# sjtuytc/UnboundedNeRFPytorch

Hardware: AMD Instinct MI355X
Metric: Msamples/sec (Mip-360 garden-shaped 1920x1080x256 frame, FourierGrid render) (higher is better)
Workload: dtype f32; 1 GPU; S1 1920x1080x256 G200 F3(P7) C12 rgbnet 39-128-128-3 f32 stepsize 1.31 thres 1e-4 white-noise grids; rays=2073600, samples_per_ray=256, chunks_per_frame=1, parallelism=1 GPU, step=ray generation + march + shade + un-tiling to image order; 3 frames in flight

## Files before the change

unboundednerfpytorch_amd/csrc/ugrid_march.hip:

```cpp
#include "ugrid_render.h"
#include "ugrid_rays.h"

__global__ void k_pack_bricks(const float *__restrict__ grid, int P, int C, int X, int Y, int Z, int H,
                              int CH, int coef, float *__restrict__ out, int64_t total) {
  for (int64_t o = (int64_t)blockIdx.x * blockDim.x + threadIdx.x; o < total;
       o += (int64_t)gridDim.x * blockDim.x) {
    int64_t q = o;
    int ch, c;
    if (H == 2) {
      const int qi = (int)(q % (8 * CH)); q /= (8 * CH);
      c = (qi >> 1) & 7;
      ch = (qi >> 4) * 2 + (qi & 1);
    } else {
      ch = (int)(q % CH); q /= CH;
      c = (int)(q % 8); q /= 8;
    }
    const int h = (int)(q % H); q /= H;
    const int k = (int)(q % (Z - 1)); q /= (Z - 1);
    const int j = (int)(q % (Y - 1)); q /= (Y - 1);
    const int i = (int)(q % (X - 1)); q /= (X - 1);
    const int l = (int)q;
    const int chan = h * CH + ch;
    float v = 0.f;
    if (chan < C) {
// ... 703 lines not shown
extern "C" int ugrid_train_sample(const float *density_grid, int P, int X, int Y, int Z, int freq_num, const float *rays_o,
                                  const float *rays_d, int64_t n_rays, const float *t_table, int32_t n_samples,
                                  const float *scene_center3, const float *scene_radius3, const float *xyz_min,
                                  const float *xyz_max, double bg_len, int norm_l2, float act_shift, float interval,
                                  float thres, float *scratch_pts, float *scratch_density, int32_t *scratch_step,
                                  float *scratch_w, float *scratch_T, int32_t *count, int32_t *count2, float *alphainv_last,
                                  ugrid_stream_t s) {
  if (!scratch_w || !scratch_T || !count2 || !alphainv_last) return (int)hipErrorInvalidValue;
  return ug_train_march_any(density_grid, P, X, Y, Z, freq_num, rays_o, rays_d, n_rays, t_table, n_samples, scene_center3, scene_radius3,
                            xyz_min, xyz_max, bg_len, norm_l2, act_shift, interval, thres, scratch_pts, scratch_density, scratch_step,
                            count, scratch_w, scratch_T, count2, alphainv_last, s);
}

extern "C" int ugrid_train_sample_compact(int64_t n_rays, int32_t n_samples, float act_shift, float interval, float thres,
                                          const float *scratch_pts, const float *scratch_density, const int32_t *scratch_step,
                                          const float *scratch_w, const float *scratch_T, const int32_t *count,
                                          const int64_t *offset_end, const int32_t *count2, const int64_t *offset_end2,
                                          const float *t_table, float *pts1, float *density1, float *weights1, float *T1,
                                          int32_t *pos2, float *pts2, float *density2, float *alpha2, float *weights2,
                                          int64_t *ray_id2, int64_t *step_id2, float *t2, ugrid_stream_t s) {
  if (n_rays <= 0) return 0;
  hipLaunchKernelGGL(k_train_compact2, dim3(ug_blocks(n_rays * UG_WAVE, 256)), dim3(256), 0, ST(s), n_rays, n_samples, act_shift, interval,
                     thres, scratch_pts, scratch_density, scratch_step, scratch_w, scratch_T, count, offset_end, count2, offset_end2,
                     t_table, pts1, density1, weights1, T1, pos2, pts2, density2, alpha2, weights2, ray_id2, step_id2, t2,
                     (uint8_t *)nullptr, ug_tl_devn.cap > 0 ? ug_tl_devn.cap : INT64_MAX);
  UG_LAUNCH_CHECK();
  return 0;
}

static int ug_fill_train_vox(ug_train_vox *v, const uint8_t *mask, const int32_t *mask_dims3, const float *xyz2ijk_scale3,
                             const float *xyz2ijk_shift3) {
  if (!mask_dims3) return (int)hipErrorInvalidValue;
  v->dist_thres = 0.f; v->near = 0.f; v->far = 0.f; v->stepdist = 1.f;
  v->plane_shift = nullptr; v->D = 1;
  return ug_fill_mask_args(*v, mask, mask_dims3[0], mask_dims3[1], mask_dims3[2], xyz2ijk_scale3, xyz2ijk_shift3);
}

extern "C" int ugrid_train_sample_dcvgo(const float *density_grid, int X, int Y, int Z, const float *rays_o, const float *rays_d,
                                        int64_t n_rays, const float *t_table, int32_t n_samples, const float *scene_center3,
                                        const float *scene_radius3, const float *xyz_min, const float *xyz_max, double bg_len,
                                        int norm_l2, float dist_thres, const uint8_t *mask, const int32_t *mask_dims3,
                                        const float *xyz2ijk_scale3, const float *xyz2ijk_shift3, float act_shift, float interval,
                                        float thres, float *scratch_pts, float *scratch_density, int32_t *scratch_step,
                                        float *scratch_w, float *scratch_T, int32_t *count, int32_t *count2, float *alphainv_last,
                                        ugrid_stream_t s) {
  if (n_rays <= 0) return 0;
  if (n_samples <= 0 || !scratch_w || !scratch_T || !count2 || !alphainv_last || !t_table) return (int)hipErrorInvalidValue;
  ug_train_vox v;
  const int rc = ug_fill_train_vox(&v, mask, mask_dims3, xyz2ijk_scale3, xyz2ijk_shift3);
  if (rc) return rc;
  v.dist_thres = dist_thres;
  ug_train_args a;
  a.n_rays = n_rays; a.S = n_samples; a.P = 1; a.F = 0; a.X = X; a.Y = Y; a.Z = Z; a.norm_l2 = norm_l2;
  a.cx = scene_center3[0]; a.cy = scene_center3[1]; a.cz = scene_center3[2];
  a.rx = scene_radius3[0]; a.ry = scene_radius3[1]; a.rz = scene_radius3[2];
  const double Bd = 1.0 + bg_len;
  a.B = (float)Bd; a.A = (float)bg_len;
  a.shift = act_shift; a.interval = interval; a.thres = thres;
  hipLaunchKernelGGL(HIP_KERNEL_NAME(k_train_march_vox<1>), dim3(ug_blocks(n_rays * UG_WAVE, 256)), dim3(256), 0, ST(s), a, v, density_grid,
                     rays_o, rays_d, t_table, xyz_min, xyz_max, scratch_pts, scratch_density, scratch_step, count, scratch_w, scratch_T,
                     count2, alphainv_last);
  UG_LAUNCH_CHECK();
  return 0;
}

extern "C" int ugrid_train_sample_dvgo(const float *density_grid, int X, int Y, int Z, const float *rays_o, const float *rays_d,
                                       int64_t n_rays, int32_t slots_per_ray, const float *xyz_min, const float *xyz_max, float near,
                                       float far, float stepdist, const uint8_t *mask, const int32_t *mask_dims3,
                                       const float *xyz2ijk_scale3, const float *xyz2ijk_shift3, float act_shift, float interval,
                                       float thres, float *scratch_pts, float *scratch_density, int32_t *scratch_step,
                                       float *scratch_w, float *scratch_T, int32_t *count, int32_t *count2, float *alphainv_last,
                                       ugrid_stream_t s) {
  if (n_rays <= 0) return 0;
  if (slots_per_ray <= 0 || !(stepdist > 0.f) || !scratch_w || !scratch_T || !count2 || !alphainv_last) return (int)hipErrorInvalidValue;
  ug_train_vox v;
  const int rc = ug_fill_train_vox(&v, mask, mask_dims3, xyz2ijk_scale3, xyz2ijk_shift3);
  if (rc) return rc;
  v.near = near; v.far = far; v.stepdist = stepdist;
  ug_train_args a;
  a.n_rays = n_rays; a.S = slots_per_ray; a.P = 1; a.F = 0; a.X = X; a.Y = Y; a.Z = Z; a.norm_l2 = 0;
  a.cx = a.cy = a.cz = 0.f; a.rx = a.ry = a.rz = 1.f; a.B = 1.f; a.A = 0.f;
  a.shift = act_shift; a.interval = interval; a.thres = thres;
  hipLaunchKernelGGL(HIP_KERNEL_NAME(k_train_march_vox<2>), dim3(ug_blocks(n_rays * UG_WAVE, 256)), dim3(256), 0, ST(s), a, v, density_grid,
                     rays_o, rays_d, (const float *)nullptr, xyz_min, xyz_max, scratch_pts, scratch_density, scratch_step, count, scratch_w,
                     scratch_T, count2, alphainv_last);
  UG_LAUNCH_CHECK();
  return 0;
}

extern "C" int ugrid_train_sample_mpi(const float *density_grid, int X, int Y, int Z, const float *rays_o, const float *rays_d,
                                      int64_t n_rays, int32_t n_steps, const float *xyz_min, const float *xyz_max,
                                      const float *act_shift, int32_t mpi_depth, const uint8_t *mask, const int32_t *mask_dims3,
                                      const float *xyz2ijk_scale3, const float *xyz2ijk_shift3, float interval, float thres,
                                      float *scratch_pts, float *scratch_density, int32_t *scratch_step, float *scratch_w,
                                      float *scratch_T, int32_t *count, int32_t *count2, float *alphainv_last, ugrid_stream_t s) {
  if (n_rays <= 0) return 0;
  if (n_steps < 2 || !act_shift || mpi_depth < 1 || mpi_depth > 256 || !scratch_w || !scratch_T || !count2 || !alphainv_last)
    return (int)hipErrorInvalidValue;
  ug_train_vox v;
  const int rc = ug_fill_train_vox(&v, mask, mask_dims3, xyz2ijk_scale3, xyz2ijk_shift3);
  if (rc) return rc;
  v.plane_shift = act_shift; v.D = mpi_depth;
  ug_train_args a;
  a.n_rays = n_rays; a.S = n_steps; a.P = 1; a.F = 0; a.X = X; a.Y = Y; a.Z = Z; a.norm_l2 = 0;
  a.cx = a.cy = a.cz = 0.f; a.rx = a.ry = a.rz = 1.f; a.B = 1.f; a.A = 0.f;
  a.shift = 0.f; a.interval = interval; a.thres = thres;
  hipLaunchKernelGGL(HIP_KERNEL_NAME(k_train_march_vox<3>), dim3(ug_blocks(n_rays * UG_WAVE, 256)), dim3(256), 0, ST(s), a, v, density_grid,
                     rays_o, rays_d, (const float *)nullptr, xyz_min, xyz_max, scratch_pts, scratch_density, scratch_step, count, scratch_w,
                     scratch_T, count2, alphainv_last);
  UG_LAUNCH_CHECK();
  return 0;
}

extern "C" int ugrid_train_sample_compact_vox(int64_t n_rays, int32_t slots_per_ray, float act_shift, float interval, float thres,
                                              const float *scratch_pts, const float *scratch_density, const int32_t *scratch_step,
                                              const float *scratch_w, const float *scratch_T, const int32_t *count,
                                              const int64_t *offset_end, const int32_t *count2, const int64_t *offset_end2,
                                              const float *t_table, float *pts1, float *density1, float *weights1, float *T1,
                                              int32_t *pos2, float *pts2, float *density2, float *alpha2, float *weights2,
                                              int64_t *ray_id2, int64_t *step_id2, float *t2, uint8_t *inner2, ugrid_stream_t s) {
  if (n_rays <= 0) return 0;
  hipLaunchKernelGGL(k_train_compact2, dim3(ug_blocks(n_rays * UG_WAVE, 256)), dim3(256), 0, ST(s), n_rays, slots_per_ray, act_shift,
                     interval, thres, scratch_pts, scratch_density, scratch_step, scratch_w, scratch_T, count, offset_end, count2,
                     offset_end2, t_table, pts1, density1, weights1, T1, pos2, pts2, density2, alpha2, weights2, ray_id2, step_id2, t2,
                     inner2, ug_tl_devn.cap > 0 ? ug_tl_devn.cap : INT64_MAX);
  UG_LAUNCH_CHECK();
  return 0;
}

extern "C" int ugrid_train_sample_backward(int64_t n_rays, float act_shift, float interval, const float *density1,
                                           const float *weights1, const float *T1, const int32_t *pos2, const int32_t *count,
                                           const int64_t *offset_end, const float *alphainv_last, const float *g_weights2,
                                           const float *g_alphainv_last, const float *g_density2, float *g_density1,
                                           ugrid_stream_t s) {
  if (n_rays <= 0) return 0;
  hipLaunchKernelGGL(k_train_sample_bwd, dim3(ug_blocks(n_rays * UG_WAVE, 256)), dim3(256), 0, ST(s), n_rays, act_shift, interval,
                     density1, weights1, T1, pos2, count, offset_end, alphainv_last, g_weights2, g_alphainv_last, g_density2, g_density1);
  UG_LAUNCH_CHECK();
  return 0;
}

extern "C" int ugrid_train_compact(int64_t n_rays, int32_t n_samples, const float *scratch_pts, const float *scratch_density,
                                   const int32_t *scratch_step, const int32_t *count, const int64_t *offset_end,
                                   const float *t_table, float *pts, float *density, int64_t *ray_id, int64_t *step_id,
                                   float *t, ugrid_stream_t s) {
  if (n_rays <= 0) return 0;
  hipLaunchKernelGGL(k_train_compact, dim3(ug_blocks(n_rays * UG_WAVE, 256)), dim3(256), 0, ST(s), n_rays, n_samples,
                     scratch_pts, scratch_density, scratch_step, count, offset_end, t_table, pts, density, ray_id, step_id, t);
  UG_LAUNCH_CHECK();
  return 0;
}

template <class MarchTile>
__device__ __forceinline__ void ug_march_block(const ug_ws_view &ws, int64_t nblocks, MarchTile march) {
  const int64_t blk = ug_xcd_remap(blockIdx.x, nblocks);
  if (blk >= nblocks) return;
  const int64_t tile = blk * 4 + (threadIdx.x >> 6);
  if (tile >= ws.n_tiles) return;
  const int n = march(tile, ws.ent + tile * ws.cap, ws.slot + tile * ws.cap);
  if (ug_lane() == 0) ws.count[tile] = n;
}

struct ug_march_geom { ug_ws_view ws; int64_t nblocks; dim3 grid; };
static inline ug_march_geom ug_march_geometry(void *ws_mem, int64_t n_rays, int32_t S) {
  ug_march_geom g;
  g.ws = ug_ws_make(ws_mem, n_rays, S);
  g.nblocks = (g.ws.n_tiles + 3) / 4;
  g.grid = dim3((unsigned)(((g.nblocks + 7) / 8) * 8));
  return g;
}

template <int F, bool L2, int W>
__global__ void __launch_bounds__(256, W)
k_march(ug_march_args a, const float *__restrict__ rays_o, const float *__restrict__ rays_d,
        const float *__restrict__ t_table, const float *__restrict__ s_table,
        const float *__restrict__ bricks, float *__restrict__ alphainv_last, float *__restrict__ depth,
        ug_ws_view ws, int64_t nblocks) {
  ug_march_block(ws, nblocks, [&](int64_t tile, float4 *ent, uint8_t *slot) {
    return ug_march_tile<F, L2>(a, rays_o, rays_d, t_table, s_table, bricks, alphainv_last, depth, tile, ent, slot);
  });
}


template <bool L2>
__global__ void __launch_bounds__(256, 5)
k_march_dcvgo(ug_march_args a, ug_dc_args dc, const float *__restrict__ rays_o, const float *__restrict__ rays_d,
              const float *__restrict__ t_table, const float *__restrict__ s_table, const float *__restrict__ bricks,
              float *__restrict__ alphainv_last, float *__restrict__ depth, float *__restrict__ wsum_mid, ug_ws_view ws,
              int64_t nblocks) {
  ug_march_block(ws, nblocks, [&](int64_t tile, float4 *ent, uint8_t *slot) {
    return ug_march_tile<0, L2, true>(a, rays_o, rays_d, t_table, s_table, bricks, alphainv_last, depth, tile, ent, slot, dc, wsum_mid);
  });
}

__global__ void __launch_bounds__(256, 6)
k_march_dvgo(ug_march_args a, ug_dv_args dv, const float *__restrict__ rays_o, const float *__restrict__ rays_d,
             const float *__restrict__ bricks, float *__restrict__ alphainv_last, float *__restrict__ depth, ug_ws_view ws,
             int64_t nblocks) {
  ug_march_block(ws, nblocks, [&](int64_t tile, float4 *ent, uint8_t *slot) {
    return ug_march_tile_dvgo(a, dv, rays_o, rays_d, bricks, alphainv_last, depth, tile, ent, slot, a.S);
  });
}

__global__ void __launch_bounds__(256, 6)
k_march_mpi(ug_march_args a, ug_mpi_args mp, const float *__restrict__ rays_o, const float *__restrict__ rays_d,
            const float *__restrict__ bricks, const float *__restrict__ act_shift, float *__restrict__ alphainv_last,
            float *__restrict__ depth, ug_ws_view ws, int64_t nblocks) {
  __shared__ float shift[256];
  if ((int)threadIdx.x < mp.D) shift[threadIdx.x] = act_shift[threadIdx.x];
  __syncthreads();
  ug_march_block(ws, nblocks, [&](int64_t tile, float4 *ent, uint8_t *slot) {
    return ug_march_tile_mpi(a, mp, rays_o, rays_d, bricks, shift, alphainv_last, depth, tile, ent, slot);
  });
}

extern "C" int64_t ugrid_render_ws_bytes(int64_t n_rays, int32_t S) {
  const int64_t n_tiles = (n_rays + UG_WAVE - 1) / UG_WAVE, cap = (int64_t)UG_WAVE * S;
  return 256 + ug_align256(n_tiles * 4) + ug_align256(n_tiles * cap * 16) + ug_align256(n_tiles * cap);
}

static int ug_grid_query_any(bool cl, const float *grid, int P, int C, int X, int Y, int Z, const float *xyz,
                             const float *xyz_min, const float *xyz_max, int freq_num, int64_t n, float *out, hipStream_t st) {
  if (n <= 0) return 0;
  if (P != (freq_num > 0 ? 2 * freq_num + 1 : 1)) return (int)hipErrorInvalidValue;
  const int64_t nl = ug_launch_rows(n);
  if (cl)
    hipLaunchKernelGGL(HIP_KERNEL_NAME(k_grid_query<true>), dim3(ug_blocks(nl * C, 256)), dim3(256), 0, st, grid, P, C, X, Y, Z, xyz,
                       xyz_min, xyz_max, freq_num, n, out, ug_tl_devn.ptr);
  else
    hipLaunchKernelGGL(HIP_KERNEL_NAME(k_grid_query<false>), dim3(ug_blocks(nl, 256)), dim3(256), 0, st, grid, P, C, X, Y, Z, xyz,
                       xyz_min, xyz_max, freq_num, n, out, ug_tl_devn.ptr);
  UG_LAUNCH_CHECK();
  return 0;
}

extern "C" int ugrid_grid_query(const float *grid, int P, int C, int X, int Y, int Z, const float *xyz,
                                const float *xyz_min, const float *xyz_max, int freq_num, int64_t n,
                                float *out, ugrid_stream_t s) {
  return ug_grid_query_any(false, grid, P, C, X, Y, Z, xyz, xyz_min, xyz_max, freq_num, n, out, ST(s));
}

extern "C" int ugrid_grid_query_cl(const float *grid, int P, int C, int X, int Y, int Z, const float *xyz,
                                   const float *xyz_min, const float *xyz_max, int freq_num, int64_t n,
                                   float *out, ugrid_stream_t s) {
  return ug_grid_query_any(true, grid, P, C, X, Y, Z, xyz, xyz_min, xyz_max, freq_num, n, out, ST(s));
}

static int ug_grid_query_backward_any(bool cl, const float *grad_out, int P, int C, int X, int Y, int Z, const float *xyz,
                                      const float *xyz_min, const float *xyz_max, int freq_num, int64_t n,
                                      float *grad_grid, hipStream_t st, uint32_t *touch = nullptr) {
  if (n <= 0) return 0;
  if (P != (freq_num > 0 ? 2 * freq_num + 1 : 1)) return (int)hipErrorInvalidValue;
  const int64_t nl = ug_launch_rows(n);
  if (cl)
    hipLaunchKernelGGL(HIP_KERNEL_NAME(k_grid_query_backward<true>), dim3(ug_blocks(nl * P * C, 256)), dim3(256), 0, st, grad_out, P, C,
                       X, Y, Z, xyz, xyz_min, xyz_max, freq_num, n, grad_grid, touch, ug_tl_devn.ptr);
  else
    hipLaunchKernelGGL(HIP_KERNEL_NAME(k_grid_query_backward<false>), dim3(ug_blocks(nl * P, 256)), dim3(256), 0, st, grad_out, P, C,
                       X, Y, Z, xyz, xyz_min, xyz_max, freq_num, n, grad_grid, (uint32_t *)nullptr, ug_tl_devn.ptr);
  UG_LAUNCH_CHECK();
  return 0;
}

extern "C" int ugrid_grid_query_backward(const float *grad_out, int P, int C, int X, int Y, int Z, const float *xyz,
                                         const float *xyz_min, const float *xyz_max, int freq_num, int64_t n,
                                         float *grad_grid, ugrid_stream_t s) {
  return ug_grid_query_backward_any(false, grad_out, P, C, X, Y, Z, xyz, xyz_min, xyz_max, freq_num, n, grad_grid, ST(s));
}

extern "C" int ugrid_grid_query_backward_cl(const float *grad_out, int P, int C, int X, int Y, int Z, const float *xyz,
                                            const float *xyz_min, const float *xyz_max, int freq_num, int64_t n,
                                            float *grad_grid, ugrid_stream_t s) {
  return ug_grid_query_backward_any(true, grad_out, P, C, X, Y, Z, xyz, xyz_min, xyz_max, freq_num, n, grad_grid, ST(s));
}

extern "C" int ugrid_grid_query_backward_cl_touch(const float *grad_out, int P, int C, int X, int Y, int Z, const float *xyz,
                                                  const float *xyz_min, const float *xyz_max, int freq_num, int64_t n,
                                                  float *grad_grid, uint32_t *touch, ugrid_stream_t s) {
  return ug_grid_query_backward_any(true, grad_out, P, C, X, Y, Z, xyz, xyz_min, xyz_max, freq_num, n, grad_grid, ST(s), touch);
}

extern "C" int ugrid_count_views_accumulate(const float *rays_o, const float *rays_d, int64_t n_rays, const float *xyz_min,
                                            const float *xyz_max, float near, float far, float stepdist, int32_t n_samples, int X, int Y,
                                            int Z, float *acc, ugrid_stream_t s) {
  if (n_rays <= 0 || n_samples <= 0) return 0;
  if (!rays_o || !rays_d || !xyz_min || !xyz_max || !acc || X < 1 || Y < 1 || Z < 1) return (int)hipErrorInvalidValue;
  hipLaunchKernelGGL(k_count_views_accumulate, dim3(ug_blocks(n_rays, 64)), dim3(64), 0, ST(s), rays_o, rays_d, n_rays, xyz_min, xyz_max,
                     near, far, stepdist, n_samples, X, Y, Z, acc);
  UG_LAUNCH_CHECK();
  return 0;
}

extern "C" int ugrid_count_views_commit(float *acc, float *count, int64_t n, ugrid_stream_t s) {
  if (n <= 0) return 0;
  if (!acc || !count) return (int)hipErrorInvalidValue;
  const int64_t blocks = ug_blocks(n, 256);
  hipLaunchKernelGGL(k_count_views_commit, dim3((unsigned)(blocks < 65536 ? blocks : 65536)), dim3(256), 0, ST(s), acc, count, n);
  UG_LAUNCH_CHECK();
  return 0;
}

static inline int ug_brick_ch(int C, int *H) {
  if (C == 1) { *H = 1; return 1; }
  *H = 2;
  return UG_CH(C);
}

extern "C" int64_t ugrid_brick_bytes(int P, int C, int X, int Y, int Z, int direct) {
  int H, CH = ug_brick_ch(C, &H);
  if (direct) { H = 1; CH = 4; }
  return (int64_t)P * (X - 1) * (Y - 1) * (Z - 1) * H * 8 * CH * (int64_t)sizeof(float);
}

extern "C" int ugrid_pack_bricks(const float *grid, int P, int C, int X, int Y, int Z, int direct,
                                 float *bricks, ugrid_stream_t s) {
  if (X < 2 || Y < 2 || Z < 2 || P < 1 || C < 1) return (int)hipErrorInvalidValue;
  int H, CH = ug_brick_ch(C, &H);
  if (direct) { H = 1; CH = 4; }
  const int64_t total = (int64_t)P * (X - 1) * (Y - 1) * (Z - 1) * H * 8 * CH;
  int64_t blocks = (total + 255) / 256;
  if (blocks > 256 * 64) blocks = 256 * 64;
  if (C == 12 && !direct) {
    if (P > 1 && (int64_t)(X - 1) * (Y - 1) * (Z - 1) * 384 >= ((int64_t)1 << 32)) return (int)hipErrorInvalidValue;
    hipLaunchKernelGGL(k_pack_quad, dim3((unsigned)blocks), dim3(256), 0, ST(s), grid, P, C, X, Y, Z, bricks, total);
    UG_LAUNCH_CHECK();
    return 0;
  }
  int coef = direct ? 0 : 1;
  hipLaunchKernelGGL(k_pack_bricks, dim3((unsigned)blocks), dim3(256), 0, ST(s), grid, P, C, X, Y, Z, H, CH,
                     coef, bricks, total);
  UG_LAUNCH_CHECK();
  return 0;
}

static int g_march_waves = 6;
extern "C" int ug_set_march_waves(int w) { if (w < 4 || w > 6) return 1; g_march_waves = w; return 0; }

template <int F, int W>
static int ug_march_launch_w(const ugrid_render_params *p, const ug_march_args &a, const float *rays_o,
                             const float *rays_d, const float *t_table, const float *s_table,
                             const float *bricks, float *alphainv_last, float *depth, const ug_march_geom &g,
                             hipStream_t st) {
  if (p->norm_l2)
    hipLaunchKernelGGL(HIP_KERNEL_NAME(k_march<F, true, W>), g.grid, dim3(256), 0, st, a, rays_o,
                       rays_d, t_table, s_table, bricks, alphainv_last, depth, g.ws, g.nblocks);
  else
    hipLaunchKernelGGL(HIP_KERNEL_NAME(k_march<F, false, W>), g.grid, dim3(256), 0, st, a, rays_o,
                       rays_d, t_table, s_table, bricks, alphainv_last, depth, g.ws, g.nblocks);
  UG_LAUNCH_CHECK();
  return 0;
}

template <int F>
static int ug_march_launch(const ugrid_render_params *p, const ug_march_args &a, const float *rays_o,
                           const float *rays_d, const float *t_table, const float *s_table,
                           const float *bricks, float *alphainv_last, float *depth, const ug_march_geom &g,
                           hipStream_t st) {
  switch (g_march_waves) {
    case 4: return ug_march_launch_w<F, 4>(p, a, rays_o, rays_d, t_table, s_table, bricks, alphainv_last, depth, g, st);
    case 6: return ug_march_launch_w<F, 6>(p, a, rays_o, rays_d, t_table, s_table, bricks, alphainv_last, depth, g, st);
    default: return ug_march_launch_w<F, 5>(p, a, rays_o, rays_d, t_table, s_table, bricks, alphainv_last, depth, g, st);
  }
}

extern "C" int ugrid_render_march(const ugrid_render_params *p, const float *rays_o, const float *rays_d,
// ... 81 lines not shown
```

unboundednerfpytorch_amd/csrc/ugrid_render.h:

```cpp
#pragma once
#include "ugrid_common.h"
#include "ugrid_math.h"
#include <string.h>

#define UG_CH(C) (2 * (((C) + 3) / 4))
#define UG_MAX_F 5


typedef float f32x16 __attribute__((ext_vector_type(16)));

struct ug_vec3 { float x, y, z; };

__device__ __forceinline__ float ug_norm3_torch(float x, float y, float z) {
  return sqrtf(fmaf(z, z, fmaf(y, y, x * x)));
}

template <bool L2>
__device__ __forceinline__ ug_vec3 ug_contract(ug_vec3 p, float B, float A) {
  const float nrm = L2 ? ug_norm3_torch(p.x, p.y, p.z) : fmaxf(fabsf(p.x), fmaxf(fabsf(p.y), fabsf(p.z)));
  if (!(nrm <= 1.0f)) {
    const float sc = B - (1.0f / nrm) * A;
    p.x = p.x / nrm * sc;
    p.y = p.y / nrm * sc;
    p.z = p.z / nrm * sc;
// ... 4 lines not shown
struct ug_axis { int cell; float wlo, whi; };

__device__ __forceinline__ ug_axis ug_axis_setup(float c, int n) {
  const float ix = ((c + 1.f) / 2.f) * (float)(n - 1);
  const float f0 = floorf(ix);
  ug_axis a;
  float wlo = (f0 + 1.f) - ix;
  float whi = ix - f0;
  int i0 = (int)fminf(fmaxf(f0, -2.f), (float)n);
  if (i0 < 0 || i0 > n - 1) wlo = 0.f;
  if (i0 + 1 < 0 || i0 + 1 > n - 1) whi = 0.f;
  if (i0 < 0) {
    a.cell = 0; a.wlo = (i0 == -1) ? whi : 0.f; a.whi = 0.f;
  } else if (i0 > n - 2) {
    a.cell = n - 2; a.whi = (i0 == n - 1) ? wlo : 0.f; a.wlo = 0.f;
  } else {
    a.cell = i0; a.wlo = wlo; a.whi = whi;
  }
  return a;
}

struct ug_cellw { int64_t rec; float w[8]; };

__device__ __forceinline__ ug_cellw ug_cell_setup(float ux, float uy, float uz, int X, int Y, int Z,
                                                 int64_t level_base) {
  const ug_axis ax = ug_axis_setup(ux, X), ay = ug_axis_setup(uy, Y), az = ug_axis_setup(uz, Z);
  ug_cellw r;
  r.rec = level_base + ((int64_t)ax.cell * (Y - 1) + ay.cell) * (Z - 1) + az.cell;
  r.w[0] = az.wlo * ay.wlo * ax.wlo;
  r.w[1] = az.whi * ay.wlo * ax.wlo;
  r.w[2] = az.wlo * ay.whi * ax.wlo;
  r.w[3] = az.whi * ay.whi * ax.wlo;
  r.w[4] = az.wlo * ay.wlo * ax.whi;
  r.w[5] = az.whi * ay.wlo * ax.whi;
  r.w[6] = az.wlo * ay.whi * ax.whi;
  r.w[7] = az.whi * ay.whi * ax.whi;
  return r;
}

template <int F>
struct ug_levels { float cx[2 * F + 1], cy[2 * F + 1], cz[2 * F + 1]; };

template <int F>
__device__ __forceinline__ ug_levels<F> ug_pe(float ux, float uy, float uz) {
  ug_levels<F> L;
  L.cx[0] = ux; L.cy[0] = uy; L.cz[0] = uz;
#pragma unroll
  for (int k = 0; k < F; ++k) {
    const float f = (float)(1 << k);
    float s, c;
    sincosf(f * ux, &s, &c); L.cx[2 * k + 1] = s; L.cx[2 * k + 2] = c;
    sincosf(f * uy, &s, &c); L.cy[2 * k + 1] = s; L.cy[2 * k + 2] = c;
    sincosf(f * uz, &s, &c); L.cz[2 * k + 1] = s; L.cz[2 * k + 2] = c;
  }
  return L;
}

__device__ __forceinline__ float ug_unorm(float p, float lo, float hi) {
  return ((p - lo) / (hi - lo)) * 2.f - 1.f;
}

struct ug_ws_view {
  int32_t *count;
  float4 *ent;
  uint8_t *slot;
  int64_t n_tiles, cap;
};
#define UG_FEAT_STRIDE 12

__host__ __device__ static inline int64_t ug_align256(int64_t x) { return (x + 255) & ~(int64_t)255; }

static inline ug_ws_view ug_ws_make(void *ws, int64_t n_rays, int32_t S) {
  ug_ws_view v;
  v.n_tiles = (n_rays + UG_WAVE - 1) / UG_WAVE;
  v.cap = (int64_t)UG_WAVE * S;
  char *b = (char *)ws + 256;
  v.count = (int32_t *)b;
  b += ug_align256(v.n_tiles * (int64_t)sizeof(int32_t));
  v.ent = (float4 *)b;
  b += ug_align256(v.n_tiles * v.cap * (int64_t)sizeof(float4));
  v.slot = (uint8_t *)b;
  return v;
}

__device__ __forceinline__ int64_t ug_xcd_remap(int64_t b, int64_t nblocks) {
  const int64_t per = (nblocks + 7) / 8;
  return (b % 8) * per + b / 8;
}

struct ug_march_args {
  int64_t n_rays;
  int32_t S, X, Y, Z;
  float cx, cy, cz, rx, ry, rz;
  float lox, loy, loz, hix, hiy, hiz;
  float ex, ey, ez, irx, iry, irz;
  float B, A;
  float shift, interval, thres;
};

__device__ __forceinline__ float ug_density_level(const char *__restrict__ lvl, float cx, float cy, float cz,
                                                  int X, int Y, int Z) {
  const ug_axis_fast ax = ug_axis_inrange(cx, X), ay = ug_axis_inrange(cy, Y), az = ug_axis_inrange(cz, Z);
  const unsigned row = (unsigned)fmaf(ax.cellf, (float)(Y - 1), ay.cellf);
  const unsigned off = __umul24(row, (unsigned)(Z - 1) << 5) + ((unsigned)az.cell << 5);
  const float4 *b = (const float4 *)(lvl + off);
  const float4 v0 = b[0], v1 = b[1];
  const float tz = az.whi, ty = ay.whi, tx = ax.whi;
  const float p00 = fmaf(v0.y, tz, v0.x), p01 = fmaf(v0.w, tz, v0.z);
  const float p10 = fmaf(v1.y, tz, v1.x), p11 = fmaf(v1.w, tz, v1.z);
  return fmaf(fmaf(p11, ty, p10), tx, fmaf(p01, ty, p00));
}

__device__ __forceinline__ void ug_normalise(const ug_march_args &a, float px, float py, float pz, float &ux, float &uy, float &uz) {
  ux = ug_div_r(px - a.lox, a.ex, a.irx) * 2.f - 1.f;
  uy = ug_div_r(py - a.loy, a.ey, a.iry) * 2.f - 1.f;
  uz = ug_div_r(pz - a.loz, a.ez, a.irz) * 2.f - 1.f;
}

__device__ __forceinline__ bool ug_outside_box(const ug_march_args &a, float px, float py, float pz) {
  return (a.lox > px) | (a.loy > py) | (a.loz > pz) | (a.hix < px) | (a.hiy < py) | (a.hiz < pz);
}

struct ug_mask_args {
  const uint8_t *mask;
  int32_t mi, mj, mk;
  float sx, sy, sz, hx, hy, hz;
};

__device__ __forceinline__ bool ug_mask_lookup(const ug_mask_args &m, float px, float py, float pz) {
  float fi = roundf(px * m.sx + m.hx), fj = roundf(py * m.sy + m.hy), fk = roundf(pz * m.sz + m.hz);
  fi = (fi != fi) ? 0.f : fi; fj = (fj != fj) ? 0.f : fj; fk = (fk != fk) ? 0.f : fk;
  if (fi >= 0.f && fi < (float)m.mi && fj >= 0.f && fj < (float)m.mj && fk >= 0.f && fk < (float)m.mk)
    return m.mask[((int64_t)fi * m.mj + (int64_t)fj) * m.mk + (int64_t)fk] != 0;
  return false;
}

static inline int ug_fill_mask_args(ug_mask_args &m, const uint8_t *mask, int32_t mask_x, int32_t mask_y, int32_t mask_z,
                                    const float *scale3, const float *shift3) {
  if (!mask || !scale3 || !shift3 || mask_x < 1 || mask_y < 1 || mask_z < 1) return (int)hipErrorInvalidValue;
  m.mask = mask; m.mi = mask_x; m.mj = mask_y; m.mk = mask_z;
  m.sx = scale3[0]; m.sy = scale3[1]; m.sz = scale3[2];
  m.hx = shift3[0]; m.hy = shift3[1]; m.hz = shift3[2];
  return 0;
}

__device__ __forceinline__ bool ug_composite(float alpha, float thres, float &T, float &w, bool &done) {
  if (!(alpha > thres)) return false;
  w = T * alpha;
  T = (float)((double)T * (1. - (double)alpha));
  if ((double)T < 1e-3) done = true;
  return w > thres;
}

__device__ __forceinline__ void ug_append_survivors(bool surv, float px, float py, float pz, float w, int lane,
                                                    float4 *__restrict__ ent, uint8_t *__restrict__ slot, int &nsurv) {
  const unsigned long long m = __ballot(surv);
  if (m != 0ull) {
    if (surv) {
      const int idx = nsurv + __builtin_amdgcn_mbcnt_hi((unsigned)(m >> 32), __builtin_amdgcn_mbcnt_lo((unsigned)m, 0u));
      ent[idx] = make_float4(px, py, pz, w);
      slot[idx] = (uint8_t)lane;
    }
    nsurv += __popcll(m);
  }
}

struct ug_dc_args : ug_mask_args {
  float dist_thres;
};

template <int F, bool L2, bool DC = false>
__device__ __forceinline__ int ug_march_tile(const ug_march_args &a, const float *__restrict__ rays_o,
                                             const float *__restrict__ rays_d, const float *__restrict__ t_table,
                                             const float *__restrict__ s_table, const float *__restrict__ bricks,
                                             float *__restrict__ alphainv_last, float *__restrict__ depth,
                                             int64_t tile, float4 *__restrict__ ent, uint8_t *__restrict__ slot,
                                             const ug_dc_args &dc = ug_dc_args{}, float *__restrict__ wsum_mid = nullptr) {
  constexpr int P = 2 * F + 1;
  const int lane = ug_lane();
  const int64_t ray = tile * UG_WAVE + lane;
  const bool valid = ray < a.n_rays;

  float ox = 0.f, oy = 0.f, oz = 0.f, dx = 0.f, dy = 0.f, dz = 1.f;
  if (valid) {
    const float rox = rays_o[3 * ray], roy = rays_o[3 * ray + 1], roz = rays_o[3 * ray + 2];
    const float rdx = rays_d[3 * ray], rdy = rays_d[3 * ray + 1], rdz = rays_d[3 * ray + 2];
    ox = (rox - a.cx) / a.rx; oy = (roy - a.cy) / a.ry; oz = (roz - a.cz) / a.rz;
    const float dn = ug_norm3_torch(rdx, rdy, rdz);
    dx = rdx / dn; dy = rdy / dn; dz = rdz / dn;
  }

  const size_t lvl_bytes = (size_t)(a.X - 1) * (a.Y - 1) * (a.Z - 1) * 32;
  const char *__restrict__ bkb = (const char *)bricks;

  float T = 1.f, dsum = 0.f;
  bool done = !valid;
  int nsurv = 0;
  [[maybe_unused]] float cum = 0.f, ppx = 0.f, ppy = 0.f, ppz = 0.f, wmid = 0.f;

  for (int j = 0; j < a.S; ++j) {
    if (__ballot(!done) == 0ull) break;
    bool surv = false;
    float w = 0.f;
    float px = 0.f, py = 0.f, pz = 0.f;
    if (!done) {
      const float t = t_table[j];
      px = ox + dx * t; py = oy + dy * t; pz = oz + dz * t;
      const float nrm = L2 ? ug_norm3_torch(px, py, pz) : fmaxf(fabsf(px), fmaxf(fabsf(py), fabsf(pz)));
      if (!(nrm <= 1.0f)) {
        const float rn = ug_rcp_refined(nrm);
        const float sc = a.B - rn * a.A;
        px = ug_div_r(px, nrm, rn) * sc;
        py = ug_div_r(py, nrm, rn) * sc;
        pz = ug_div_r(pz, nrm, rn) * sc;
      }
      float ux, uy, uz;
      ug_normalise(a, px, py, pz, ux, uy, uz);
      bool keep = true;
      [[maybe_unused]] bool inner = true;
      if constexpr (DC) {
        inner = nrm <= 1.0f;
        keep = inner;
        if (j > 0) {
          cum += ug_norm3_torch(px - ppx, py - ppy, pz - ppz);
          const bool over = cum > dc.dist_thres;
          cum *= over ? 0.f : 1.f;
          keep = keep || over;
        }
        ppx = px; ppy = py; ppz = pz;
        if (keep) keep = ug_mask_lookup(dc, px, py, pz);
      }
      if (keep) {
        float dens = ug_density_level(bkb, ux, uy, uz, a.X, a.Y, a.Z);
#pragma unroll
        for (int k = 0; k < F; ++k) {
          const float f = (float)(1 << k);
          float sx, cx_, sy, cy_, sz, cz_;
          if (k == 0) {
            ug_sincos_small(ux, &sx, &cx_);
            ug_sincos_small(uy, &sy, &cy_);
            ug_sincos_small(uz, &sz, &cz_);
          } else {
            ug_sincos(f * ux, &sx, &cx_);
            ug_sincos(f * uy, &sy, &cy_);
            ug_sincos(f * uz, &sz, &cz_);
          }
          dens += ug_density_level(bkb + (size_t)(2 * k + 1) * lvl_bytes, sx, sy, sz, a.X, a.Y, a.Z);
          dens += ug_density_level(bkb + (size_t)(2 * k + 2) * lvl_bytes, cx_, cy_, cz_, a.X, a.Y, a.Z);
        }
        dens = ug_div_r(dens, (float)P, 1.0f / (float)P);
        const float xs = dens + a.shift;
        const float alpha = ug_alpha(xs, a.interval);
        if (alpha > a.thres) {
          w = T * alpha;
          T = (float)((double)T * (1. - (double)alpha));
          if (w > a.thres) {
            surv = true;
            dsum += w * s_table[j];
            if constexpr (DC) { if (inner) wmid += w; }
          }
          if ((double)T < 1e-3) done = true;
        }
      }
    }
    ug_append_survivors(surv, px, py, pz, w, lane, ent, slot, nsurv);
  }
  if (valid) {
    alphainv_last[ray] = T;
    depth[ray] = dsum;
    if constexpr (DC) wsum_mid[ray] = wmid;
  }
  return nsurv;
}

struct ug_dv_args : ug_mask_args {
  float near, far, stepdist;
};

__device__ __forceinline__ int ug_march_tile_dvgo(const ug_march_args &a, const ug_dv_args &dv, const float *__restrict__ rays_o,
                                                  const float *__restrict__ rays_d, const float *__restrict__ bricks,
                                                  float *__restrict__ alphainv_last, float *__restrict__ depth, int64_t tile,
                                                  float4 *__restrict__ ent, uint8_t *__restrict__ slot, int cap) {
  const int lane = ug_lane();
  const int64_t ray = tile * UG_WAVE + lane;
  const bool valid = ray < a.n_rays;
  float sx = 0.f, sy = 0.f, sz = 0.f, dx = 0.f, dy = 0.f, dz = 0.f;
  int n = 0;
  if (valid) {
    const float ox = rays_o[3 * ray], oy = rays_o[3 * ray + 1], oz = rays_o[3 * ray + 2];
    const float rx = rays_d[3 * ray], ry = rays_d[3 * ray + 1], rz = rays_d[3 * ray + 2];
    const float vx = (rx == 0.f) ? (float)1e-6 : rx, vy = (ry == 0.f) ? (float)1e-6 : ry, vz = (rz == 0.f) ? (float)1e-6 : rz;
    const float ax = (a.hix - ox) / vx, ay = (a.hiy - oy) / vy, az = (a.hiz - oz) / vz;
    const float bx = (a.lox - ox) / vx, by = (a.loy - oy) / vy, bz = (a.loz - oz) / vz;
    const float tmin = fmaxf(fminf(fmaxf(fmaxf(fminf(ax, bx), fminf(ay, by)), fminf(az, bz)), dv.far), dv.near);
    const float tmax = fmaxf(fminf(fminf(fminf(fmaxf(ax, bx), fmaxf(ay, by)), fmaxf(az, bz)), dv.far), dv.near);
    const float rn = sqrtf(rx * rx + ry * ry + rz * rz);
    const double c = (double)ceilf((tmax - tmin) * rn / dv.stepdist);
    const double nn = c > 1. ? c : 1.;
    n = nn > (double)cap ? cap : (int)nn;
    sx = ox + rx * tmin; sy = oy + ry * tmin; sz = oz + rz * tmin;
    dx = rx / rn; dy = ry / rn; dz = rz / rn;
  }
  const char *__restrict__ bkb = (const char *)bricks;
  float T = 1.f, dsum = 0.f;
  bool done = !valid;
  int nsurv = 0;
  for (int j = 0;; ++j) {
    done = done || j >= n;
    if (__ballot(!done) == 0ull) break;
    bool surv = false;
    float w = 0.f, px = 0.f, py = 0.f, pz = 0.f;
    if (!done) {
      const float dist = dv.stepdist * (float)j;
      px = sx + dx * dist; py = sy + dy * dist; pz = sz + dz * dist;
      if (!ug_outside_box(a, px, py, pz) && ug_mask_lookup(dv, px, py, pz)) {
        float ux, uy, uz;
        ug_normalise(a, px, py, pz, ux, uy, uz);
        const float dens = ug_density_level(bkb, ux, uy, uz, a.X, a.Y, a.Z);
        surv = ug_composite(ug_alpha(dens + a.shift, a.interval), a.thres, T, w, done);
        if (surv) dsum += w * (float)j;
      }
    }
    ug_append_survivors(surv, px, py, pz, w, lane, ent, slot, nsurv);
  }
  if (valid) {
    alphainv_last[ray] = T;
    depth[ray] = dsum;
  }
  return nsurv;
}

struct ug_mpi_args : ug_mask_args {
  int32_t D, n;
};

__device__ __forceinline__ int ug_march_tile_mpi(const ug_march_args &a, const ug_mpi_args &mp, const float *__restrict__ rays_o,
                                                 const float *__restrict__ rays_d, const float *__restrict__ bricks,
                                                 const float *__restrict__ shift, float *__restrict__ alphainv_last,
                                                 float *__restrict__ depth, int64_t tile, float4 *__restrict__ ent,
                                                 uint8_t *__restrict__ slot) {
  const int lane = ug_lane();
  const int64_t ray = tile * UG_WAVE + lane;
  const bool valid = ray < a.n_rays;
  float ox = 0.f, oy = 0.f, oz = 0.f, rx = 0.f, ry = 0.f, rz = 0.f;
  if (valid) {
    ox = rays_o[3 * ray]; oy = rays_o[3 * ray + 1]; oz = rays_o[3 * ray + 2];
    rx = rays_d[3 * ray]; ry = rays_d[3 * ray + 1]; rz = rays_d[3 * ray + 2];
  }
  const char *__restrict__ bkb = (const char *)bricks;
  const float dm1 = (float)(mp.D - 1), nm1 = (float)(mp.n - 1), nf = (float)mp.n;
  float T = 1.f, dsum = 0.f;
  bool done = !valid;
  int nsurv = 0;
  for (int j = 0; j < mp.n; ++j) {
    if (__ballot(!done) == 0ull) break;
    bool surv = false;
    float w = 0.f, px = 0.f, py = 0.f, pz = 0.f;
    if (!done) {
      const float dist = (float)j / nm1;
      px = ox + rx * dist; py = oy + ry * dist; pz = oz + rz * dist;
      if (!ug_outside_box(a, px, py, pz) && ug_mask_lookup(mp, px, py, pz)) {
        float ux, uy, uz;
        ug_normalise(a, px, py, pz, ux, uy, uz);
        const float dens = ug_density_level(bkb, ux, uy, uz, a.X, a.Y, a.Z);
        const float iz = ((uz + 1.f) / 2.f) * dm1;
        const float f0 = floorf(iz);
        const int i0 = min(max((int)f0, 0), mp.D - 1);
        float sh = shift[i0] * ((f0 + 1.f) - iz);
        if (i0 + 1 < mp.D) sh = sh + shift[i0 + 1] * (iz - f0);
        surv = ug_composite(ug_alpha(dens + sh, a.interval), a.thres, T, w, done);
        if (surv) dsum += w * (((float)j + 0.5f) / nf);
      }
    }
    ug_append_survivors(surv, px, py, pz, w, lane, ent, slot, nsurv);
  }
  if (valid) {
    alphainv_last[ray] = T;
    depth[ray] = dsum;
  }
  return nsurv;
}

__host__ __device__ static inline int ug_feat_of(int o, int r, int h) { return 32 * o + (r & 3) + 8 * (r >> 2) + 4 * h; }

struct ug_mlp_layout { int KL, offA1, offA2, offB1, offB2, offW3, offb3, total;
                       int KB1, bfA1, bfA2, bfB1, bfB2, bfW3, bfb3, total2;
                       int hxA1, hxA2, hxB1, hxB2, hxW3, hxb3, hxS, total3; };
struct ug_mlp_scales { float sX1, sW1, sX2, sW2; };
__host__ __device__ static inline ug_mlp_layout ug_mlp_lay(int C, int n_emb) {
  const int CH = UG_CH(C);
  ug_mlp_layout L;
  L.KL = (2 * CH + n_emb + 1) / 2;
  L.offA1 = 0;
  L.offA2 = L.offA1 + L.KL * 256;
  L.offB1 = L.offA2 + 64 * 256;
  L.offB2 = L.offB1 + 128;
  L.offW3 = L.offB2 + 128;
  L.offb3 = L.offW3 + 512;
  L.total = L.offb3 + 4;
  L.KB1 = (L.KL + 7) / 8;
  L.bfA1 = L.total;
  L.bfA2 = L.bfA1 + L.KB1 * 4 * 3 * 64 * 4;
  L.bfB1 = L.bfA2 + 8 * 4 * 3 * 64 * 4;
  L.bfB2 = L.bfB1 + 128;
  L.bfW3 = L.bfB2 + 128;
  L.bfb3 = L.bfW3 + 512;
  L.total2 = L.bfb3 + 4;
  L.hxA1 = L.total2;
  L.hxA2 = L.hxA1 + L.KB1 * 4 * 2 * 64 * 4;
  L.hxB1 = L.hxA2 + 8 * 4 * 2 * 64 * 4;
  L.hxB2 = L.hxB1 + 128;
  L.hxW3 = L.hxB2 + 128;
  L.hxb3 = L.hxW3 + 512;
  L.hxS = L.hxb3 + 4;
  L.total3 = L.hxS + 4;
  return L;
}

__host__ __device__ static inline int ug_in_col(int s, int h, int C, int n_emb, int KL) {
  const int CH = UG_CH(C);
  if (s < CH) {
    const int ch = h * CH + s;
    return ch < C ? ch : -1;
  }
  const int e = h * (KL - CH) + (s - CH);
  return e < n_emb ? C + e : -1;
}

#ifndef UG_K0_BATCH
#define UG_K0_BATCH 2
#endif

struct ug_shade_args {
  int64_t n_rays;
  int32_t X, Y, Z;
  int32_t residual;
  float lox, loy, loz, hix, hiy, hiz;
  float ex, ey, ez, irx, iry, irz;
};

struct ug_k0_cell { const float4 *rec; float tx, ty, tz; };
template <int CH>
__device__ __forceinline__ ug_k0_cell ug_k0_cell_setup(const float *__restrict__ k0b, int h, int64_t level_base, float cx,
                                                       float cy, float cz, int X, int Y, int Z) {
  const ug_axis_fast ax = ug_axis_inrange(cx, X), ay = ug_axis_inrange(cy, Y), az = ug_axis_inrange(cz, Z);
  const unsigned row = (unsigned)fmaf(ax.cellf, (float)(Y - 1), ay.cellf);
  const unsigned cell = __umul24(row, (unsigned)(Z - 1)) + (unsigned)az.cell;
  ug_k0_cell c;
  c.rec = (const float4 *)(k0b + ((level_base + cell) * 2 + h) * (8 * CH));
  c.tx = ax.whi; c.ty = ay.whi; c.tz = az.whi;
  return c;
}

template <int F, int CH>
__device__ __forceinline__ void ug_k0_gather(const float *__restrict__ k0b, int h, float px, float py, float pz,
                                             const ug_shade_args &a, float (&feat)[CH]) {
  constexpr int P = 2 * F + 1;
  constexpr int NB = UG_K0_BATCH;
  static_assert((8 * CH) % 4 == 0, "half-brick must be a whole number of float4");
  const float ux = ug_div_r(px - a.lox, a.ex, a.irx) * 2.f - 1.f;
  const float uy = ug_div_r(py - a.loy, a.ey, a.iry) * 2.f - 1.f;
  const float uz = ug_div_r(pz - a.loz, a.ez, a.irz) * 2.f - 1.f;
  const int64_t cells = (int64_t)(a.X - 1) * (a.Y - 1) * (a.Z - 1);
  ug_k0_cell c[P];
  c[0] = ug_k0_cell_setup<CH>(k0b, h, 0, ux, uy, uz, a.X, a.Y, a.Z);
#pragma unroll
  for (int k = 0; k < F; ++k) {
    const float f = (float)(1 << k);
    float sx, cx_, sy, cy_, sz, cz_;
    ug_sincos(f * ux, &sx, &cx_);
    ug_sincos(f * uy, &sy, &cy_);
    ug_sincos(f * uz, &sz, &cz_);
    c[2 * k + 1] = ug_k0_cell_setup<CH>(k0b, h, (int64_t)(2 * k + 1) * cells, sx, sy, sz, a.X, a.Y, a.Z);
    c[2 * k + 2] = ug_k0_cell_setup<CH>(k0b, h, (int64_t)(2 * k + 2) * cells, cx_, cy_, cz_, a.X, a.Y, a.Z);
  }
#pragma unroll
  for (int s = 0; s < CH; ++s) feat[s] = 0.f;
#pragma unroll
  for (int b0 = 0; b0 < P; b0 += NB) {
    float4 v[NB][2 * CH];
#pragma unroll
    for (int l = 0; l < NB; ++l)
      if (b0 + l < P) {
#pragma unroll
        for (int q = 0; q < 2 * CH; ++q) v[l][q] = c[b0 + l].rec[q];
      }
    __builtin_amdgcn_sched_barrier(0);
#pragma unroll
    for (int l = 0; l < NB; ++l)
      if (b0 + l < P) {
        const float tz = c[b0 + l].tz, ty = c[b0 + l].ty, tx = c[b0 + l].tx;
#pragma unroll
        for (int pr = 0; pr < CH / 2; ++pr) {
          const float4 q0 = v[l][4 * pr], q1 = v[l][4 * pr + 1], q2 = v[l][4 * pr + 2], q3 = v[l][4 * pr + 3];
          const float a00 = fmaf(q0.z, tz, q0.x), a01 = fmaf(q1.z, tz, q1.x);
          const float a10 = fmaf(q2.z, tz, q2.x), a11 = fmaf(q3.z, tz, q3.x);
          const float b00 = fmaf(q0.w, tz, q0.y), b01 = fmaf(q1.w, tz, q1.y);
          const float b10 = fmaf(q2.w, tz, q2.y), b11 = fmaf(q3.w, tz, q3.y);
          const float fa = fmaf(fmaf(a11, ty, a10), tx, fmaf(a01, ty, a00));
          const float fb = fmaf(fmaf(b11, ty, b10), tx, fmaf(b01, ty, b00));
          feat[2 * pr] = (b0 + l == 0) ? fa : feat[2 * pr] + fa;
          feat[2 * pr + 1] = (b0 + l == 0) ? fb : feat[2 * pr + 1] + fb;
        }
      }
  }
#pragma unroll
  for (int ch = 0; ch < CH; ++ch) feat[ch] = ug_div_r(feat[ch], (float)P, 1.0f / (float)P);
}

typedef float ug_f4 __attribute__((ext_vector_type(4)));
template <int IMM>
__device__ __forceinline__ ug_f4 ug_gload4(unsigned voff, const float *sbase) {
  ug_f4 r;
  asm volatile("global_load_dwordx4 %0, %1, %2 offset:%3" : "=v"(r) : "v"(voff), "s"(sbase), "n"(IMM) : "memory");
  return r;
}
template <int IMM>
__device__ __forceinline__ ug_f4 ug_gload4v(const char *vaddr) {
  ug_f4 r;
  asm volatile("global_load_dwordx4 %0, %1, off offset:%2" : "=v"(r) : "v"(vaddr), "n"(IMM) : "memory");
  return r;
}
template <int N>
__device__ __forceinline__ void ug_vmwait6(ug_f4 (&v)[6]) {
  asm volatile("s_waitcnt vmcnt(%6)" : "+v"(v[0]), "+v"(v[1]), "+v"(v[2]), "+v"(v[3]), "+v"(v[4]), "+v"(v[5]) : "n"(N));
}

template <int K>
// ... 962 lines not shown
```

Before: 63540 Msamples/s.

## Stage march survivors in per-wave LDS ring and flush coalesced 64-entry chunks

Survivor samples from the march loop were scattered straight to global memory, with each step writing a few float4 entries and slot bytes at irregular offsets. They now go into a per-wave 128-entry shared-memory ring buffer and are written to global in full 64-entry chunks, coalesced by lane, plus a final partial flush. This is meant to cut the partial-line and byte-sized global stores of the compaction path. The cost is about 8.5KB of LDS per block, which may lower occupancy given the launch bounds of 5-6 blocks, plus wave barriers and extra LDS traffic.

Measured after the change: 63600 Msamples/s (median of 6 runs). About the same (+0.1%).

```diff
diff --git a/unboundednerfpytorch_amd/csrc/ugrid_march.hip b/unboundednerfpytorch_amd/csrc/ugrid_march.hip
--- a/unboundednerfpytorch_amd/csrc/ugrid_march.hip
+++ b/unboundednerfpytorch_amd/csrc/ugrid_march.hip
@@ -879,12 +879,13 @@
 }
 
 template <class MarchTile>
-__device__ __forceinline__ void ug_march_block(const ug_ws_view &ws, int64_t nblocks, MarchTile march) {
+__device__ __forceinline__ void ug_march_block(const ug_ws_view &ws, int64_t nblocks, ug_ring *rings, MarchTile march) {
   const int64_t blk = ug_xcd_remap(blockIdx.x, nblocks);
   if (blk >= nblocks) return;
-  const int64_t tile = blk * 4 + (threadIdx.x >> 6);
+  const int wave = __builtin_amdgcn_readfirstlane((int)(threadIdx.x >> 6));
+  const int64_t tile = blk * 4 + wave;
   if (tile >= ws.n_tiles) return;
-  const int n = march(tile, ws.ent + tile * ws.cap, ws.slot + tile * ws.cap);
+  const int n = march(tile, rings + wave, ws.ent + tile * ws.cap, ws.slot + tile * ws.cap);
   if (ug_lane() == 0) ws.count[tile] = n;
 }
 
@@ -903,8 +904,9 @@
         const float *__restrict__ t_table, const float *__restrict__ s_table,
         const float *__restrict__ bricks, float *__restrict__ alphainv_last, float *__restrict__ depth,
         ug_ws_view ws, int64_t nblocks) {
-  ug_march_block(ws, nblocks, [&](int64_t tile, float4 *ent, uint8_t *slot) {
-    return ug_march_tile<F, L2>(a, rays_o, rays_d, t_table, s_table, bricks, alphainv_last, depth, tile, ent, slot);
+  __shared__ ug_ring rings[4];
+  ug_march_block(ws, nblocks, rings, [&](int64_t tile, ug_ring *ring, float4 *ent, uint8_t *slot) {
+    return ug_march_tile<F, L2>(a, rays_o, rays_d, t_table, s_table, bricks, alphainv_last, depth, tile, ring, ent, slot);
   });
 }
 
@@ -915,8 +917,9 @@
               const float *__restrict__ t_table, const float *__restrict__ s_table, const float *__restrict__ bricks,
               float *__restrict__ alphainv_last, float *__restrict__ depth, float *__restrict__ wsum_mid, ug_ws_view ws,
               int64_t nblocks) {
-  ug_march_block(ws, nblocks, [&](int64_t tile, float4 *ent, uint8_t *slot) {
-    return ug_march_tile<0, L2, true>(a, rays_o, rays_d, t_table, s_table, bricks, alphainv_last, depth, tile, ent, slot, dc, wsum_mid);
+  __shared__ ug_ring rings[4];
+  ug_march_block(ws, nblocks, rings, [&](int64_t tile, ug_ring *ring, float4 *ent, uint8_t *slot) {
+    return ug_march_tile<0, L2, true>(a, rays_o, rays_d, t_table, s_table, bricks, alphainv_last, depth, tile, ring, ent, slot, dc, wsum_mid);
   });
 }
 
@@ -924,8 +927,9 @@
 k_march_dvgo(ug_march_args a, ug_dv_args dv, const float *__restrict__ rays_o, const float *__restrict__ rays_d,
              const float *__restrict__ bricks, float *__restrict__ alphainv_last, float *__restrict__ depth, ug_ws_view ws,
              int64_t nblocks) {
-  ug_march_block(ws, nblocks, [&](int64_t tile, float4 *ent, uint8_t *slot) {
-    return ug_march_tile_dvgo(a, dv, rays_o, rays_d, bricks, alphainv_last, depth, tile, ent, slot, a.S);
+  __shared__ ug_ring rings[4];
+  ug_march_block(ws, nblocks, rings, [&](int64_t tile, ug_ring *ring, float4 *ent, uint8_t *slot) {
+    return ug_march_tile_dvgo(a, dv, rays_o, rays_d, bricks, alphainv_last, depth, tile, ring, ent, slot, a.S);
   });
 }
 
@@ -936,8 +940,9 @@
   __shared__ float shift[256];
   if ((int)threadIdx.x < mp.D) shift[threadIdx.x] = act_shift[threadIdx.x];
   __syncthreads();
-  ug_march_block(ws, nblocks, [&](int64_t tile, float4 *ent, uint8_t *slot) {
-    return ug_march_tile_mpi(a, mp, rays_o, rays_d, bricks, shift, alphainv_last, depth, tile, ent, slot);
+  __shared__ ug_ring rings[4];
+  ug_march_block(ws, nblocks, rings, [&](int64_t tile, ug_ring *ring, float4 *ent, uint8_t *slot) {
+    return ug_march_tile_mpi(a, mp, rays_o, rays_d, bricks, shift, alphainv_last, depth, tile, ring, ent, slot);
   });
 }
 
diff --git a/unboundednerfpytorch_amd/csrc/ugrid_render.h b/unboundednerfpytorch_amd/csrc/ugrid_render.h
--- a/unboundednerfpytorch_amd/csrc/ugrid_render.h
+++ b/unboundednerfpytorch_amd/csrc/ugrid_render.h
@@ -180,17 +180,39 @@
   return w > thres;
 }
 
+#define UG_RING 128
+struct ug_ring { float4 ent[UG_RING]; uint8_t slot[UG_RING]; };
+
+__device__ __forceinline__ void ug_ring_flush(ug_ring *__restrict__ ring, int base, int n, int lane, float4 *__restrict__ ent,
+                                              uint8_t *__restrict__ slot) {
+  __builtin_amdgcn_wave_barrier();
+  if (lane < n) {
+    const int i = base + lane;
+    ent[i] = ring->ent[i & (UG_RING - 1)];
+    slot[i] = ring->slot[i & (UG_RING - 1)];
+  }
+  __builtin_amdgcn_wave_barrier();
+}
+
 __device__ __forceinline__ void ug_append_survivors(bool surv, float px, float py, float pz, float w, int lane,
-                                                    float4 *__restrict__ ent, uint8_t *__restrict__ slot, int &nsurv) {
+                                                    ug_ring *__restrict__ ring, float4 *__restrict__ ent,
+                                                    uint8_t *__restrict__ slot, int &nsurv) {
   const unsigned long long m = __ballot(surv);
   if (m != 0ull) {
     if (surv) {
       const int idx = nsurv + __builtin_amdgcn_mbcnt_hi((unsigned)(m >> 32), __builtin_amdgcn_mbcnt_lo((unsigned)m, 0u));
-      ent[idx] = make_float4(px, py, pz, w);
-      slot[idx] = (uint8_t)lane;
-    }
-    nsurv += __popcll(m);
-  }
+      ring->ent[idx & (UG_RING - 1)] = make_float4(px, py, pz, w);
+      ring->slot[idx & (UG_RING - 1)] = (uint8_t)lane;
+    }
+    const int total = nsurv + __popcll(m);
+    if ((total >> 6) != (nsurv >> 6)) ug_ring_flush(ring, nsurv & ~63, 64, lane, ent, slot);
+    nsurv = total;
+  }
+}
+
+__device__ __forceinline__ void ug_flush_survivors(ug_ring *__restrict__ ring, int lane, float4 *__restrict__ ent,
+                                                   uint8_t *__restrict__ slot, int nsurv) {
+  if (nsurv & 63) ug_ring_flush(ring, nsurv & ~63, nsurv & 63, lane, ent, slot);
 }
 
 struct ug_dc_args : ug_mask_args {
@@ -202,8 +224,8 @@
                                              const float *__restrict__ rays_d, const float *__restrict__ t_table,
                                              const float *__restrict__ s_table, const float *__restrict__ bricks,
                                              float *__restrict__ alphainv_last, float *__restrict__ depth,
-                                             int64_t tile, float4 *__restrict__ ent, uint8_t *__restrict__ slot,
-                                             const ug_dc_args &dc = ug_dc_args{}, float *__restrict__ wsum_mid = nullptr) {
+                                             int64_t tile, ug_ring *__restrict__ ring, float4 *__restrict__ ent,
+                                             uint8_t *__restrict__ slot, const ug_dc_args &dc = ug_dc_args{}, float *__restrict__ wsum_mid = nullptr) {
   constexpr int P = 2 * F + 1;
   const int lane = ug_lane();
   const int64_t ray = tile * UG_WAVE + lane;
@@ -291,8 +313,9 @@
         }
       }
     }
-    ug_append_survivors(surv, px, py, pz, w, lane, ent, slot, nsurv);
-  }
+    ug_append_survivors(surv, px, py, pz, w, lane, ring, ent, slot, nsurv);
+  }
+  ug_flush_survivors(ring, lane, ent, slot, nsurv);
   if (valid) {
     alphainv_last[ray] = T;
     depth[ray] = dsum;
@@ -308,7 +331,8 @@
 __device__ __forceinline__ int ug_march_tile_dvgo(const ug_march_args &a, const ug_dv_args &dv, const float *__restrict__ rays_o,
                                                   const float *__restrict__ rays_d, const float *__restrict__ bricks,
                                                   float *__restrict__ alphainv_last, float *__restrict__ depth, int64_t tile,
-                                                  float4 *__restrict__ ent, uint8_t *__restrict__ slot, int cap) {
+                                                  ug_ring *__restrict__ ring, float4 *__restrict__ ent, uint8_t *__restrict__ slot,
+                                                  int cap) {
   const int lane = ug_lane();
   const int64_t ray = tile * UG_WAVE + lane;
   const bool valid = ray < a.n_rays;
@@ -349,8 +373,9 @@
         if (surv) dsum += w * (float)j;
       }
     }
-    ug_append_survivors(surv, px, py, pz, w, lane, ent, slot, nsurv);
-  }
+    ug_append_survivors(surv, px, py, pz, w, lane, ring, ent, slot, nsurv);
+  }
+  ug_flush_survivors(ring, lane, ent, slot, nsurv);
   if (valid) {
     alphainv_last[ray] = T;
     depth[ray] = dsum;
@@ -365,8 +390,8 @@
 __device__ __forceinline__ int ug_march_tile_mpi(const ug_march_args &a, const ug_mpi_args &mp, const float *__restrict__ rays_o,
                                                  const float *__restrict__ rays_d, const float *__restrict__ bricks,
                                                  const float *__restrict__ shift, float *__restrict__ alphainv_last,
-                                                 float *__restrict__ depth, int64_t tile, float4 *__restrict__ ent,
-                                                 uint8_t *__restrict__ slot) {
+                                                 float *__restrict__ depth, int64_t tile, ug_ring *__restrict__ ring,
+                                                 float4 *__restrict__ ent, uint8_t *__restrict__ slot) {
   const int lane = ug_lane();
   const int64_t ray = tile * UG_WAVE + lane;
   const bool valid = ray < a.n_rays;
@@ -400,8 +425,9 @@
         if (surv) dsum += w * (((float)j + 0.5f) / nf);
       }
     }
-    ug_append_survivors(surv, px, py, pz, w, lane, ent, slot, nsurv);
-  }
+    ug_append_survivors(surv, px, py, pz, w, lane, ring, ent, slot, nsurv);
+  }
+  ug_flush_survivors(ring, lane, ent, slot, nsurv);
   if (valid) {
     alphainv_last[ray] = T;
     depth[ray] = dsum;
```
